# mcgillmrl/prob_mbrl

Measured on AMD Instinct MI355X. Metric: particle_rollouts_per_sec, higher is better.
Workload: dtype f32 via split fp16 (fwd, 2 pieces) / bf16 (adjoint, 2 pieces) MFMA, fp32 accumulate

## Files before the change

prob_mbrl_amd/csrc/pmbrl_reg.h:

```cpp
#pragma once
#include <cstddef>
#include <type_traits>
#include <utility>
#include "pmbrl_dev.h"
#include "pmbrl_split.h"
#include "pmbrl_reg_head.h"
#include "pmbrl_reg_mm.h"

#define PR_NTHR (PR_NW * 64)
#define PR_NT 13
#define PR_KB 7
#define PM_GLOBAL_ __attribute__((address_space(1)))
typedef float f32x2 __attribute__((ext_vector_type(2)));

#define PR_RES_FLOATS (PR_NW * PR_SLOTS * PR_KB * 2 * PR_FRAG)
#define PR_XT_FLOATS (PR_KB * 2 * PR_FRAG)
#define PR_L0P_FLOATS (PR_NT * 2 * PR_FRAG)
#define PR_L0_FLOATS (PR_NT * PR_FRAG)
#define PR_HEAD_FLOATS (PR_NW * 2 * 2 * PR_FRAG)
#define PR_NET_FLOATS (PR_RES_FLOATS + PR_XT_FLOATS + PR_L0P_FLOATS + PR_HEAD_FLOATS)
#define PR_OFF_RES 0
#define PR_OFF_XT (PR_RES_FLOATS)
#define PR_OFF_L0 (PR_RES_FLOATS + PR_XT_FLOATS)
#define PR_OFF_HEAD (PR_RES_FLOATS + PR_XT_FLOATS + PR_L0P_FLOATS)
// ... 203 lines not shown
      for (int e = 0; e < 8; ++e) {
        int ot = -1;
        if (blk == 0) ot = 4 * (e >> 2) + w;
        else if (e < 4) ot = 8 + w;
        else if (w == pr_xwave(net)) ot = PR_XT;
        const int k = ot >= 0 ? 16 * ot + 4 * g + (e & 3) : hid;
        piece[e] = p;
        if (k < hid) {
          if (dir == 0) {
            const int row = pr_head_row(net, P.D, P.U, m);
            if (row >= 0 && row < n_out) v[e] = W2[(size_t)row * hid + k];
          } else {
            const int i = 2 * (m >> 2) + ((m >> 1) & 1);
            if ((m & 1) == 0 && i < n_in) v[e] = W0[(size_t)k * n_in + i];
          }
        }
      }
    }
    unsigned short h[8];
#pragma unroll
    for (int e = 0; e < 8; ++e) {
      if (f16 && piece[e] == 0 && P.wflag && !(fabsf(v[e]) <= 65504.f)) atomicMax(P.wflag, P.gen);
      h[e] = pr_piece(v[e], piece[e], f16);
    }
    uint4 o4;
    o4.x = h[0] | ((unsigned)h[1] << 16);
    o4.y = h[2] | ((unsigned)h[3] << 16);
    o4.z = h[4] | ((unsigned)h[5] << 16);
    o4.w = h[6] | ((unsigned)h[7] << 16);
    *reinterpret_cast<uint4*>(P.out + ((size_t)dn * PR_NET_FLOATS + (size_t)fr * PR_FRAG) + lane * 4) = o4;
  }
}

__device__ __forceinline__ void pr_barrier() { asm volatile("s_waitcnt lgkmcnt(0)\n\ts_barrier" ::: "memory"); }
typedef __amdgpu_buffer_rsrc_t pr_rsrc;
__device__ __forceinline__ pr_rsrc pr_make_rsrc(void* base) {
  return __builtin_amdgcn_make_buffer_rsrc(base, 0, 0xffffffff, 0x00020000);
}
__device__ __forceinline__ int pr_uni(int v) { return __builtin_amdgcn_readfirstlane(v); }
#ifdef PR_EXP_NOSTASH
#define PR_EXP_STASH(x) ;
#else
#define PR_EXP_STASH(x) x
#endif
typedef int pr_i32x4 __attribute__((ext_vector_type(4)));
__device__ __forceinline__ pr_i32x4 pr_rsrc_words(const void* base) {
  const unsigned long long a = (unsigned long long)base;
  pr_i32x4 r;
  r[0] = __builtin_amdgcn_readfirstlane((int)(unsigned)a);
  r[1] = __builtin_amdgcn_readfirstlane((int)((unsigned)(a >> 32) & 0xffffu));
  r[2] = -1;
  r[3] = 0x00020000;
  return r;
}
__device__ __forceinline__ void pr_aload4_b8(unsigned (&d)[4], const pr_i32x4& srd, unsigned voff, int s0, int s1, int s2, int s3) {
  asm volatile("s_nop 4\n\tbuffer_load_ubyte %0, %4, %5, %6 offen\n\tbuffer_load_ubyte %1, %4, %5, %7 offen\n\t"
               "buffer_load_ubyte %2, %4, %5, %8 offen\n\tbuffer_load_ubyte %3, %4, %5, %9 offen"
               : "=&v"(d[0]), "=&v"(d[1]), "=&v"(d[2]), "=&v"(d[3])
               : "v"(voff), "s"(srd), "s"(s0), "s"(s1), "s"(s2), "s"(s3)
               : "memory");
}

#define PR_NRESF (2 * PR_SLOTS * PR_KB * 2)
#define PR_NAG 62
struct RegW {
  f32x4 a[PR_NAG];
  f32x4 v[PR_NRESF - PR_NAG];
};
__host__ __device__ constexpr int pr_widx(int net, int slot, int kb, int p) { return ((net * PR_SLOTS + slot) * PR_KB + kb) * 2 + p; }

template <int I>
__device__ __forceinline__ void pr_res_load(RegW& W, unsigned voff, const float* packed_dir, int wid) {
  typedef const PM_GLOBAL_ char* gcp;
  constexpr int net = I / (PR_SLOTS * PR_KB * 2), r = I % (PR_SLOTS * PR_KB * 2);
  gcp src = (gcp)(packed_dir + (size_t)net * PR_NET_FLOATS + PR_OFF_RES + ((size_t)wid * (PR_SLOTS * PR_KB * 2) + r) * PR_FRAG);
  if constexpr (I < PR_NAG) asm volatile("global_load_dwordx4 %0, %1, %2" : "=a"(W.a[I]) : "v"(voff), "s"(src) : "memory");
  else asm volatile("global_load_dwordx4 %0, %1, %2" : "=v"(W.v[I - PR_NAG]) : "v"(voff), "s"(src) : "memory");
}
template <int I>
__device__ __forceinline__ void pr_res_tie(RegW& W) {
  if constexpr (I < PR_NAG) asm volatile("" : "+a"(W.a[I]));
  else asm volatile("" : "+v"(W.v[I - PR_NAG]));
}
__device__ __forceinline__ void pr_load_resident(RegW& W, const float* packed_dir, int wid, int lane) {
  const unsigned voff = (unsigned)lane * 16u;
  pr_for<PR_NRESF>([&](auto ic) { pr_res_load<decltype(ic)::value>(W, voff, packed_dir, wid); });
  asm volatile("s_waitcnt vmcnt(0)" ::: "memory");
  pr_for<PR_NRESF>([&](auto ic) { pr_res_tie<decltype(ic)::value>(W); });
}

template <int NET, bool F16, bool XT>
__device__ __forceinline__ void pr_hidden_layer(const RegW& W, const float* lds, const float* xtw, int lane,
                                                f32x4 (&acc)[PR_SLOTS][2], f32x4 (&accx)[2]) {
  const float* act = lds + PR_LDS_ACT + lane * 4;
  f32x4 b[2][2];
  f32x4 xw[2][2];
  auto fetch = [&](int kb) {
    const int q = kb & 1;
    b[q][0] = *reinterpret_cast<const f32x4*>(act + (kb * 2 + 0) * PR_FRAG);
    b[q][1] = *reinterpret_cast<const f32x4*>(act + (kb * 2 + 1) * PR_FRAG);
    if constexpr (XT) {
      xw[q][0] = *reinterpret_cast<const f32x4*>(xtw + lane * 4 + (kb * 2 + 0) * PR_FRAG);
      xw[q][1] = *reinterpret_cast<const f32x4*>(xtw + lane * 4 + (kb * 2 + 1) * PR_FRAG);
    }
  };
  fetch(0);
  pr_for<PR_KB>([&](auto ic) {
    constexpr int kb = decltype(ic)::value;
    constexpr int q = kb & 1;
    if constexpr (kb + 1 < PR_KB) fetch(kb + 1);
    pr_for<PR_SLOTS>([&](auto sc) {
      constexpr int s = decltype(sc)::value;
      constexpr int I = pr_widx(NET, s, kb, 1);
      if constexpr (kb == 0) {
        if constexpr (I < PR_NAG) pr_mfma0<F16, true>(acc[s][0], W.a[I], b[q][0]);
        else pr_mfma0<F16, false>(acc[s][0], W.v[I - PR_NAG], b[q][0]);
      } else {
        if constexpr (I < PR_NAG) pr_mfma<F16, true>(acc[s][0], W.a[I], b[q][0]);
        else pr_mfma<F16, false>(acc[s][0], W.v[I - PR_NAG], b[q][0]);
      }
    });
    if constexpr (XT) {
      if constexpr (kb == 0) pr_mfma0<F16, false>(accx[0], xw[q][1], b[q][0]);
      else pr_mfma<F16, false>(accx[0], xw[q][1], b[q][0]);
    }
    pr_for<PR_SLOTS>([&](auto sc) {
      constexpr int s = decltype(sc)::value;
      constexpr int I = pr_widx(NET, s, kb, 0);
      if constexpr (kb == 0) {
        if constexpr (I < PR_NAG) pr_mfma0<F16, true>(acc[s][1], W.a[I], b[q][1]);
        else pr_mfma0<F16, false>(acc[s][1], W.v[I - PR_NAG], b[q][1]);
      } else {
        if constexpr (I < PR_NAG) pr_mfma<F16, true>(acc[s][1], W.a[I], b[q][1]);
        else pr_mfma<F16, false>(acc[s][1], W.v[I - PR_NAG], b[q][1]);
      }
    });
    if constexpr (XT) {
      if constexpr (kb == 0) pr_mfma0<F16, false>(accx[1], xw[q][0], b[q][1]);
      else pr_mfma<F16, false>(accx[1], xw[q][0], b[q][1]);
    }
    pr_for<PR_SLOTS>([&](auto sc) {
      constexpr int s = decltype(sc)::value;
      constexpr int I = pr_widx(NET, s, kb, 0);
      if constexpr (I < PR_NAG) pr_mfma<F16, true>(acc[s][1], W.a[I], b[q][0]);
      else pr_mfma<F16, false>(acc[s][1], W.v[I - PR_NAG], b[q][0]);
    });
    if constexpr (XT) pr_mfma<F16, false>(accx[1], xw[q][0], b[q][0]);
  });
  if constexpr (XT)
    asm volatile("s_nop 7\n\ts_nop 7" : "+v"(acc[0][0]), "+v"(acc[0][1]), "+v"(acc[1][0]), "+v"(acc[1][1]), "+v"(acc[2][0]),
                 "+v"(acc[2][1]), "+v"(accx[0]), "+v"(accx[1]));
  else
    asm volatile("s_nop 7\n\ts_nop 7" : "+v"(acc[0][0]), "+v"(acc[0][1]), "+v"(acc[1][0]), "+v"(acc[1][1]), "+v"(acc[2][0]),
                 "+v"(acc[2][1]));
}

template <bool F16>
__device__ __forceinline__ f32x4 pr_tile_value(const f32x4 (&c)[2]) {
  return pm_chains_sum<F16, 2>(c[0], c[1]);
}

template <bool F16>
__device__ __forceinline__ void pr_split(f32x4 h, pm_u32x2& hi, pm_u32x2& lo) {
  if constexpr (F16) {
    const unsigned ha = pm_pk_f16(h[0], h[1]), hb = pm_pk_f16(h[2], h[3]);
    float l0, l1, l2, l3;
    asm("v_fma_mix_f32 %0, %1, -1.0, %2 op_sel:[0,0,0] op_sel_hi:[1,0,0]" : "=v"(l0) : "v"(ha), "v"(h[0]));
    asm("v_fma_mix_f32 %0, %1, -1.0, %2 op_sel:[1,0,0] op_sel_hi:[1,0,0]" : "=v"(l1) : "v"(ha), "v"(h[1]));
    asm("v_fma_mix_f32 %0, %1, -1.0, %2 op_sel:[0,0,0] op_sel_hi:[1,0,0]" : "=v"(l2) : "v"(hb), "v"(h[2]));
    asm("v_fma_mix_f32 %0, %1, -1.0, %2 op_sel:[1,0,0] op_sel_hi:[1,0,0]" : "=v"(l3) : "v"(hb), "v"(h[3]));
    hi = pm_u32x2{ha, hb};
    lo = pm_u32x2{pm_pk_f16(l0, l1), pm_pk_f16(l2, l3)};
  } else {
    pm_u32x2 pc[2];
    pm_split4<2, F16>(h, pc);
    hi = pc[0];
    lo = pc[1];
  }
}

__device__ __forceinline__ float pr_rcp(float d) {
  const float r = __builtin_amdgcn_rcpf(d);
  return __builtin_fmaf(__builtin_fmaf(-d, r, 1.f), r, r);
}
__device__ __forceinline__ float pr_exp(float x) {
  const float t = x * 1.44269504f;
  const float eps = __builtin_fmaf(x, 1.92596299e-8f, __builtin_fmaf(x, 1.44269504f, -t));
  const float p = __builtin_amdgcn_exp2f(t);
  return __builtin_fmaf(p, eps * 0.693147181f, p);
}
__device__ __forceinline__ float pr_tanh(float u) {
  const float r = 1.f - 2.f * pr_rcp(1.f + pr_exp(2.f * __builtin_amdgcn_fmed3f(u, -15.f, 15.f)));
  return u != u ? u : r;
}
__device__ __forceinline__ float pr_sigmoid_neg(float y) { return pr_rcp(1.f + pr_exp(__builtin_amdgcn_fmed3f(y, -80.f, 80.f))); }

template <bool F16>
__device__ __forceinline__ void pr_tile_epilogue(f32x4 v, f32x4 mf, f32x4& h, unsigned& ab, unsigned& amax, pm_u32x2& hi,
                                                 pm_u32x2& lo) {
  const f32x4 t = v * mf;
#pragma unroll
  for (int r = 0; r < 4; ++r) h[r] = fmaxf(t[r], 0.f);
  {
    unsigned x0, x1, x2, x3;
    asm("v_min_u32 %0, 1, %1" : "=v"(x0) : "v"(__float_as_uint(h[0])));
    asm("v_min_u32 %0, 1, %1" : "=v"(x1) : "v"(__float_as_uint(h[1])));
    asm("v_min_u32 %0, 1, %1" : "=v"(x2) : "v"(__float_as_uint(h[2])));
    asm("v_min_u32 %0, 1, %1" : "=v"(x3) : "v"(__float_as_uint(h[3])));
    unsigned a01, a23;
    asm("v_lshl_or_b32 %0, %1, 1, %2" : "=v"(a01) : "v"(x1), "v"(x0));
    asm("v_lshl_or_b32 %0, %1, 1, %2" : "=v"(a23) : "v"(x3), "v"(x2));
    asm("v_lshl_or_b32 %0, %1, 2, %2" : "=v"(ab) : "v"(a23), "v"(a01));
  }
  amax = max(max(amax, max(__float_as_uint(h[0]), __float_as_uint(h[1]))), max(__float_as_uint(h[2]), __float_as_uint(h[3])));
  if constexpr (F16) {
    const unsigned ha = pm_pk_f16(h[0], h[1]), hb = pm_pk_f16(h[2], h[3]);
    float l0, l1, l2, l3;
    asm("v_fma_mix_f32 %0, %1, -1.0, %2 op_sel:[0,0,0] op_sel_hi:[1,0,0]" : "=v"(l0) : "v"(ha), "v"(h[0]));
    asm("v_fma_mix_f32 %0, %1, -1.0, %2 op_sel:[1,0,0] op_sel_hi:[1,0,0]" : "=v"(l1) : "v"(ha), "v"(h[1]));
    asm("v_fma_mix_f32 %0, %1, -1.0, %2 op_sel:[0,0,0] op_sel_hi:[1,0,0]" : "=v"(l2) : "v"(hb), "v"(h[2]));
    asm("v_fma_mix_f32 %0, %1, -1.0, %2 op_sel:[1,0,0] op_sel_hi:[1,0,0]" : "=v"(l3) : "v"(hb), "v"(h[3]));
    hi = pm_u32x2{ha, hb};
    lo = pm_u32x2{pm_pk_f16(l0, l1), pm_pk_f16(l2, l3)};
  } else {
    pm_u32x2 pc[2];
    pm_split4<2, F16>(h, pc);
    hi = pc[0];
    lo = pc[1];
  }
}

template <int L0_BLOCKS>
__device__ __forceinline__ void pr_copy_net_to_lds(float* smem, int lds_l0, int lds_xt, int lds_head, const float* src, int tid) {
  constexpr int N_L0 = PR_NT * L0_BLOCKS * PR_FRAG / 4, N_XT = PR_XT_FLOATS / 4, N_HD = PR_HEAD_FLOATS / 4;
  constexpr int I_L0 = (N_L0 + PR_NTHR - 1) / PR_NTHR, I_XT = (N_XT + PR_NTHR - 1) / PR_NTHR, I_HD = (N_HD + PR_NTHR - 1) / PR_NTHR;
  f32x4 a[I_L0], b[I_XT], c[I_HD];
#pragma unroll
  for (int k = 0; k < I_L0; ++k) {
    const int i = min(tid + k * PR_NTHR, N_L0 - 1);
    a[k] = ldg4(src + PR_OFF_L0 + (L0_BLOCKS == 1 ? (i >> 6) * (2 * PR_FRAG) + (i & 63) * 4 : i * 4));
  }
#pragma unroll
  for (int k = 0; k < I_XT; ++k) b[k] = ldg4(src + PR_OFF_XT + min(tid + k * PR_NTHR, N_XT - 1) * 4);
#pragma unroll
  for (int k = 0; k < I_HD; ++k) c[k] = ldg4(src + PR_OFF_HEAD + min(tid + k * PR_NTHR, N_HD - 1) * 4);
#pragma unroll
  for (int k = 0; k < I_L0; ++k)
    if (tid + k * PR_NTHR < N_L0) *reinterpret_cast<f32x4*>(smem + lds_l0 + (tid + k * PR_NTHR) * 4) = a[k];
#pragma unroll
  for (int k = 0; k < I_XT; ++k)
    if (tid + k * PR_NTHR < N_XT) *reinterpret_cast<f32x4*>(smem + lds_xt + (tid + k * PR_NTHR) * 4) = b[k];
#pragma unroll
  for (int k = 0; k < I_HD; ++k)
    if (tid + k * PR_NTHR < N_HD) *reinterpret_cast<f32x4*>(smem + lds_head + (tid + k * PR_NTHR) * 4) = c[k];
}

template <bool PROF, int MMD = 0, bool TREE = false>
__global__ __launch_bounds__(PR_NTHR, 1) void pm_reg_fwd_kernel(const RegArgs A) {
  extern __shared__ __attribute__((aligned(16))) float smem[];
  constexpr bool F16 = true;
  constexpr int MMDc = MMD ? MMD : 2;
  typedef PM_GLOBAL_ uint8_t gu8;
  typedef PM_GLOBAL_ float gf32;
  typedef PM_GLOBAL_ char gch;
  const int tid = threadIdx.x, lane = tid & 63;
  const int wid = __builtin_amdgcn_readfirstlane(tid >> 6);
  const int wg = pr_wg(A);
  if (wg < 0) return;
  const int row = lane & 15, g = lane >> 4;
  int row0, nvalid;
  pr_rows(A, wg, row0, nvalid);
  const bool rvalid = row < nvalid;
  const int D = A.D, U = A.U, B = A.B;
  const float* packed = A.packed;

  if (PROF && wg == 0 && tid == 0) {
    A.prof[30] = (long long)__builtin_readcyclecounter();
    A.prof[28] = (long long)__builtin_amdgcn_s_memrealtime();
  }
  float c_mx[2], c_isx[2], c_sy[2], c_my[2], c_zp[2], c_zd[2], c_psc[2], c_pbi[2];
  float x[2];
  unsigned so_x[2], so_a[2];
  bool ok_x[2], ok_a[2];
#pragma unroll
  for (int s = 0; s < 2; ++s) {
    const int i = 2 * g + s;
    const bool isd = i < D, isa = i >= D && i < D + U;
    const int ja = isa ? i - D : 0, id = isd ? i : 0;
    c_mx[s] = (isd || isa) ? A.mx[i] : 0.f;
    c_isx[s] = (isd || isa) ? A.iSx[i] : 0.f;
    c_sy[s] = isd ? A.Sy[id] : 0.f;
    c_my[s] = isd ? A.my[id] : 0.f;
    c_zp[s] = (isa && rvalid) ? A.zpol[(size_t)(row0 + row) * U + ja] : 0.f;
    c_zd[s] = (isd && rvalid) ? A.zdyn[(size_t)(row0 + row) * D + id] : 0.f;
    c_psc[s] = isa ? A.pscale[ja] : 0.f;
    c_pbi[s] = isa ? A.pbias[ja] : 0.f;
    x[s] = (isd && rvalid) ? A.x0[(size_t)(row0 + row) * D + id] : 0.f;
    ok_x[s] = isd && rvalid;
    ok_a[s] = isa && rvalid;
    so_x[s] = ((unsigned)(row0 + row) * D + id) * 4u;
    so_a[s] = ((unsigned)(row0 + row) * U + ja) * 4u;
  }
  f32x4 hbp, hbd;
#pragma unroll
  for (int r = 0; r < 4; ++r) {
    const int rp = pr_head_row(0, D, U, 4 * g + r), rd = pr_head_row(1, D, U, 4 * g + r);
    hbp[r] = rp >= 0 ? (A.pol_params + A.pol.b_off[2])[rp] : 0.f;
    hbd[r] = rd >= 0 ? (A.dyn_params + A.dyn.b_off[2])[rd] : 0.f;
  }
  unsigned mbits[2][2][PR_SLOTS + 1];
#pragma unroll
  for (int n = 0; n < 2; ++n)
#pragma unroll
    for (int l = 0; l < 2; ++l) {
      const uint16_t* mrow = (n == 0 ? A.pol : A.dyn).mask[l] + (size_t)(row0 + (rvalid ? row : 0)) * PR_NT;
#pragma unroll
      for (int q = 0; q <= PR_SLOTS; ++q) mbits[n][l][q] = (unsigned)mrow[q < PR_SLOTS ? 4 * q + wid : PR_XT];
    }
  RegW W;
  pr_load_resident(W, packed, wid, lane);
  if (PROF && wg == 0 && tid == 0) A.prof[27] = (long long)__builtin_readcyclecounter();
#pragma unroll
  for (int s = 0; s < 2; ++s)
    if (ok_x[s] && wid == 0) *(gf32*)((gch*)A.states + so_x[s]) = x[s];
  pr_copy_net_to_lds<1>(smem, PR_LDS_L0(0), PR_LDS_XT(0), PR_LDS_HEAD(0), packed, tid);
  pr_copy_net_to_lds<1>(smem, PR_LDS_L0(1), PR_LDS_XT(1), PR_LDS_HEAD(1), packed + PR_NET_FLOATS, tid);
  if (PROF && wg == 0 && tid == 0) A.prof[26] = (long long)__builtin_readcyclecounter();
  for (int i = tid; i < PR_KB * 2 * PR_FRAG; i += PR_NTHR) smem[PR_LDS_ACT + i] = 0.f;
  if (tid < 16) smem[PR_LDS_FLAG + tid] = 0.f;
#pragma unroll
  for (int n = 0; n < 2; ++n)
#pragma unroll
    for (int l = 0; l < 2; ++l) {
      const RegNet& N = n == 0 ? A.pol : A.dyn;
#pragma unroll
      for (int q = 0; q <= PR_SLOTS; ++q) {
        if (q == PR_SLOTS && wid != pr_xwave(n)) continue;
        const unsigned nib = rvalid ? ((mbits[n][l][q] >> (4 * g)) & 0xFu) : 0u;
        f32x4 mf;
#pragma unroll
        for (int r = 0; r < 4; ++r) mf[r] = ((nib >> r) & 1u) ? N.inv_keep[l] : 0.f;
        float* dst = q < PR_SLOTS ? smem + PR_LDS_MF + (size_t)(((wid * 2 + n) * 2 + l) * PR_SLOTS + q) * PR_FRAG
                                  : smem + PR_LDS_MFX + (size_t)(n * 2 + l) * PR_FRAG;
        *reinterpret_cast<f32x4*>(dst + lane * 4) = mf;
      }
    }
  __syncthreads();
  if (tid < 64) reinterpret_cast<unsigned*>(smem + PR_LDS_ACT + ((PR_KB - 1) * 2 + 0) * PR_FRAG + tid * 4)[2] = 0x3c00u;
  if (tid == 0 && A.wflag && *A.wflag == A.wgen) atomicMin(A.status, 0);
  if (PROF && wg == 0 && tid == 0) A.prof[25] = (long long)__builtin_readcyclecounter();

  bool any_a[2], any_x[2];
#pragma unroll
  for (int s = 0; s < 2; ++s) {
    any_a[s] = false;
    any_x[s] = false;
    for (int gg = 0; gg < 4; ++gg) {
      const int i = 2 * gg + s;
      any_a[s] = any_a[s] || (i >= D && i < D + U);
      any_x[s] = any_x[s] || i < D;
    }
  }
  const float max_std_pol = expf(A.mls_pol), max_std_dyn = expf(A.mls_dyn);
  const int mm_gi = MMD ? wg / A.mm.parts : 0, mm_me = MMD ? wg - mm_gi * A.mm.parts : 0, mm_g0 = mm_gi * (MMD ? A.mm.M : 0);
  double mm_ref = 0.0;
  double* const mm_zh = reinterpret_cast<double*>(smem + PR_LDS_ZH);
  double* const mm_rec = reinterpret_cast<double*>(smem + PR_LDS_REC);
  if constexpr (MMD != 0) {
    if (wid == 0) mm_ref = row < MMD ? (double)A.x0[(size_t)mm_g0 * D + row] : 0.0;
    if (wid == 1) pr_mm_fwd_prep<MMDc>(A.mm, 0, mm_gi, mm_g0, row0, nvalid, mm_me, lane, mm_zh);
  }
  unsigned amax = 0u;
  const bool xw_pol = wid == pr_xwave(0), xw_dyn = wid == pr_xwave(1);
  float* const act_w = smem + PR_LDS_ACT + lane * 4;
  const float* const mf_w = smem + PR_LDS_MF + (size_t)wid * (2 * 2 * PR_SLOTS * PR_FRAG) + lane * 4;
  const float* const mfx_w = smem + PR_LDS_MFX + lane * 4;
  const unsigned lane_st = ((4u * g) * 16u + row) * 4u;
  const pr_rsrc srd = pr_make_rsrc(A.ws);
  const unsigned vo_abp = (unsigned)lane * 4u;
  int so_abp = (wg * PR_NW + wid) * 256;
  const int abp_step = A.nwg * (PR_NW * 256);

  auto first_layer = [&](auto netc, const float (&in)[2], int so_ab, int so_st) {
    constexpr int NET = decltype(netc)::value;
    _Float16 hh[2], hl[2], hs[2];
#pragma unroll
    for (int s = 0; s < 2; ++s) {
      hh[s] = (_Float16)in[s];
      hl[s] = (_Float16)(in[s] - (float)hh[s]);
      hs[s] = hh[s] * (_Float16)PM_F16_LO_ISCALE;
      amax = max(amax, __float_as_uint(in[s]) & 0x7fffffffu);
#ifdef PR_EXP_AMAX_CODE
      if (!(fabsf(in[s]) <= 3.0e38f)) atomicMin(A.status, -((NET + 1) * 1000000 + lane * 1000 + s * 100 + wg));
#endif
    }
    const pm_f16x8 bf = {hh[0], hl[0], hs[0], hh[1], hl[1], hs[1], (_Float16)1.0f, (_Float16)PM_F16_LO_ISCALE};
    const float* l0w = smem + PR_LDS_L0(NET) + lane * 4;
    const bool xw = NET == 0 ? xw_pol : xw_dyn;
    f32x4 acc[PR_SLOTS + 1];
    const f32x4 bfv = __builtin_bit_cast(f32x4, bf);
    f32x4 wf[PR_SLOTS + 1];
    pr_for<PR_SLOTS>([&](auto qc) {
      constexpr int q = decltype(qc)::value;
      wf[q] = *reinterpret_cast<const f32x4*>(l0w + (size_t)(4 * q + wid) * PR_FRAG);
    });
    wf[PR_SLOTS] = *reinterpret_cast<const f32x4*>(l0w + (size_t)PR_XT * PR_FRAG);
    f32x4 mfv[PR_SLOTS + 1];
    pr_for<PR_SLOTS>([&](auto qc) {
      constexpr int q = decltype(qc)::value;
      mfv[q] = *reinterpret_cast<const f32x4*>(mf_w + (size_t)((NET * 2 + 0) * PR_SLOTS + q) * PR_FRAG);
    });
    mfv[PR_SLOTS] = *reinterpret_cast<const f32x4*>(mfx_w + (size_t)(NET * 2 + 0) * PR_FRAG);
    pr_mfma_open();
    pr_for<PR_SLOTS + 1>([&](auto qc) {
      constexpr int q = decltype(qc)::value;
      pr_mfma0<F16, false, true>(acc[q], wf[q], bfv);
    });
    asm volatile("s_nop 7\n\ts_nop 7" : "+v"(acc[0]), "+v"(acc[1]), "+v"(acc[2]), "+v"(acc[3]));
    unsigned abw = 0u;
    auto epi = [&](auto qc, int ot) {
      constexpr int q = decltype(qc)::value;
      f32x4 h;
      unsigned ab;
      pm_u32x2 hi, lo;
      pr_tile_epilogue<F16>(acc[q], mfv[q], h, ab, amax, hi, lo);
      float* dst = act_w + (size_t)((ot >> 1) * 2) * PR_FRAG + 2 * (ot & 1);
      *reinterpret_cast<pm_u32x2*>(dst) = hi;
      *reinterpret_cast<pm_u32x2*>(dst + PR_FRAG) = lo;
      abw |= ab << (4 * q);
      if constexpr (NET == 0) {
#pragma unroll
        for (int r = 0; r < 4; ++r)
// ... 220 lines not shown
  if (U.mm_on) {
    const int gi = wg / U.parts, me = wg - gi * U.parts;
    row0 = gi * U.M + me * U.rpw;
    nvalid = min(U.rpw, U.M - me * U.rpw);
  }
  const int rowg = row0 + (lane & 15), g = lane >> 4;
  if ((lane & 15) >= nvalid) return;
  for (int n = 0; n < 2; ++n)
    for (int l = 0; l < 2; ++l) {
      const unsigned w = U.src[n][l][((size_t)t * U.nwg + wg) * PR_NTHR + tid];
      unsigned char* d = U.dst[n][l] + ((size_t)t * U.B + rowg) * (PR_NT * 4) + g;
#pragma unroll
      for (int q = 0; q < PR_SLOTS; ++q) d[(4 * q + wid) * 4] = (unsigned char)((w >> (4 * q)) & 15u);
      if (wid == pr_xwave(n)) d[PR_XT * 4] = (unsigned char)((w >> (4 * PR_SLOTS)) & 15u);
    }
}

#define PRB_LDS_ACT 0
#define PRB_LDS_PART (PRB_LDS_ACT + PR_KB * 2 * PR_FRAG)
#define PRB_LDS_L0(net) (PRB_LDS_PART + PR_NW * PR_FRAG + (net) * (PR_L0P_FLOATS + PR_XT_FLOATS + PR_HEAD_FLOATS))
#define PRB_LDS_XT(net) (PRB_LDS_L0(net) + PR_L0P_FLOATS)
#define PRB_LDS_HEAD(net) (PRB_LDS_XT(net) + PR_XT_FLOATS)
#define PRB_LDS_LUT (PRB_LDS_L0(2))
#define PRB_IN_COLS 32
#define PRB_LDS_IN (PRB_LDS_LUT + 2 * 2 * 16 * 4)
#define PRB_LDS_XB (PRB_LDS_IN + 16 * PRB_IN_COLS)
#define PRB_LDS_MMB (PRB_LDS_XB + 128)
#define PRB_LDS_MMY (PRB_LDS_MMB + 2 * 2 * PR_MM_BOP_DOUBLES)
#define PRB_LDS_XH (PRB_LDS_MMY + 2 * 2 * PR_MM_YOP_DOUBLES(6))
#define PRB_LDS_XTAG (PRB_LDS_XH + 2 * PM_XCH_HELP_DOUBLES(2))
#define PRB_LDS_FLOATS (PRB_LDS_XTAG + 16)

template <bool PROF, int MMD = 0, bool TREE = false>
__global__ __launch_bounds__(PR_NTHR, 1) void pm_reg_bwd_kernel(const RegArgs A) {
  extern __shared__ __attribute__((aligned(16))) float smem[];
  constexpr bool F16 = false;
  constexpr int MMDc = MMD ? MMD : 2;
  typedef PM_GLOBAL_ float gf32;
  const int tid = threadIdx.x, lane = tid & 63;
  const int wid = __builtin_amdgcn_readfirstlane(tid >> 6);
  const int wg = pr_wg(A);
  if (wg < 0) return;
  const int row = lane & 15, g = lane >> 4;
  int row0, nvalid;
  pr_rows(A, wg, row0, nvalid);
  const bool rvalid = row < nvalid;
  const int D = A.D, U = A.U, B = A.B;
  const int T0 = A.t0;
  int T1 = A.t1;
  if (A.nvalid) T1 = min(T1, __builtin_amdgcn_readfirstlane(*A.nvalid));
  const float* packed = A.packed + (size_t)2 * PR_NET_FLOATS;
  if (T1 <= T0) {
    for (int i = tid; i < nvalid * D; i += PR_NTHR) {
      if (A.grad_x0 && T0 == 0) A.grad_x0[(size_t)row0 * D + i] = 0.f;
      if (A.gx_out) A.gx_out[(size_t)row0 * D + i] = A.gx_in ? A.gx_in[(size_t)row0 * D + i] : 0.f;
    }
    return;
  }

  if (PROF && wg == 0 && tid == 0) {
    A.prof[30] = (long long)__builtin_readcyclecounter();
    A.prof[28] = (long long)__builtin_amdgcn_s_memrealtime();
  }
  float c_isx[2], c_sy[2], c_psc[2], c_pbi[2];
  bool ok_x[2], ok_a[2];
  unsigned so_x[2], so_a[2];
  float gx[2] = {0.f, 0.f};
#pragma unroll
  for (int s = 0; s < 2; ++s) {
    const int i = 2 * g + s;
    const bool isd = i < D, isa = i >= D && i < D + U;
    const int ja = isa ? i - D : 0, id = isd ? i : 0;
    c_isx[s] = (isd || isa) ? A.iSx[i] : 0.f;
    c_sy[s] = isd ? A.Sy[id] : 0.f;
    c_psc[s] = isa ? A.pscale[ja] : 1.f;
    c_pbi[s] = isa ? A.pbias[ja] : 0.f;
    ok_x[s] = isd && rvalid;
    ok_a[s] = isa && rvalid;
    so_x[s] = ((unsigned)(row0 + row) * D + id) * 4u;
    so_a[s] = ((unsigned)(row0 + row) * U + ja) * 4u;
    if (A.gx_in && ok_x[s]) gx[s] = *(const gf32*)((const PM_GLOBAL_ char*)A.gx_in + so_x[s]);
  }
  RegW W;
  pr_load_resident(W, packed, wid, lane);
  pr_copy_net_to_lds<2>(smem, PRB_LDS_L0(0), PRB_LDS_XT(0), PRB_LDS_HEAD(0), packed, tid);
  pr_copy_net_to_lds<2>(smem, PRB_LDS_L0(1), PRB_LDS_XT(1), PRB_LDS_HEAD(1), packed + PR_NET_FLOATS, tid);
  for (int i = tid; i < PR_KB * 2 * PR_FRAG; i += PR_NTHR) smem[PRB_LDS_ACT + i] = 0.f;
  if (tid < 16) smem[PRB_LDS_XTAG + tid] = 0.f;
  if (tid < 64) {
    const int n = tid >> 5, l = (tid >> 4) & 1, nib = tid & 15;
    const float ik = (n == 0 ? A.pol : A.dyn).inv_keep[l];
    f32x4 m;
#pragma unroll
    for (int r = 0; r < 4; ++r) m[r] = ((nib >> r) & 1) ? ik : 0.f;
    *reinterpret_cast<f32x4*>(smem + PRB_LDS_LUT + tid * 4) = m;
  }
  __syncthreads();

  const bool xw_pol = wid == pr_xwave(0), xw_dyn = wid == pr_xwave(1);
  float* const act_w = smem + PRB_LDS_ACT + lane * 4;
  const float* const lut = smem + PRB_LDS_LUT;
  const unsigned lane_st = ((4u * g) * 16u + row) * 4u;
  const pr_rsrc srd = pr_make_rsrc(A.ws);
  const unsigned x_step = (unsigned)B * D * 4u, a_step = (unsigned)B * U * 4u;
  const int st_step = A.nwg * (PR_NT * 1024), st_step2 = A.nwg * 1024;
  int so_g0 = (int)A.gT[0] + ((T1 - 1) * A.nwg + wg) * (PR_NT * 1024);
  int so_g2 = (int)A.gT[2] + ((T1 - 1) * A.nwg + wg) * 1024;

  float* const stage = smem + PRB_LDS_IN;
  typedef const PM_GLOBAL_ char* gcp;
  gcp sp[2];
  unsigned sstep[2];
#pragma unroll
  for (int k = 0; k < 2; ++k) {
    const int e = tid + k * PR_NTHR, r = e >> 5, c = e & 31;
    const long long grow = row0 + r;
    gcp q = (gcp)A.ws;
    unsigned st = 0u;
    if (r < nvalid) {
      const int i = c >= 18 ? c - 18 : (c >= 10 ? c - 10 : c - 2);
      if (c == 0) {
        q = (gcp)A.grad_rewards + ((long long)(T1 - 1) * B + grow) * 4;
        st = (unsigned)B * 4u;
      } else if (c >= 2 && c < 26 && i < D && c < 18) {
        q = (gcp)A.ws + (c < 10 ? A.Jx : A.Td) + ((long long)(T1 - 1) * B + grow) * D * 4 + i * 4;
        st = x_step;
      } else if (c >= 2 && c < 26 && i >= D && i < D + U) {
        q = (c >= 18 ? (gcp)A.actions : (gcp)A.ws + (c < 10 ? A.Ja : A.Tp)) + ((long long)(T1 - 1) * B + grow) * U * 4 + (i - D) * 4;
        st = a_step;
      }
    }
    sp[k] = q;
    sstep[k] = st;
  }
  float sv[2];
  auto stage_load = [&]() {
    asm volatile("global_load_dword %0, %2, off\n\tglobal_load_dword %1, %3, off" : "=&v"(sv[0]), "=&v"(sv[1]) : "v"(sp[0]), "v"(sp[1]) : "memory");
  };
  auto stage_landed = [&](auto nc, float (&v)[2]) {
    constexpr int N = decltype(nc)::value;
    asm volatile("s_waitcnt vmcnt(%2)" : "+v"(v[0]), "+v"(v[1]) : "n"(N) : "memory");
  };
  auto stage_park = [&]() {
    stage[tid] = sv[0];
    stage[tid + PR_NTHR] = sv[1];
  };
  const pr_i32x4 wsrd = pr_rsrc_words(A.ws);
  const unsigned vo_abp = (unsigned)lane * 4u;
  const int abp_step = A.nwg * (PR_NW * 256);
  int so_abp = ((T1 - 1) * A.nwg + wg) * (PR_NW * 256) + wid * 256;
  auto ab_load = [&](unsigned (&w)[4]) {
    asm volatile("s_nop 4\n\tbuffer_load_dword %0, %4, %5, %6 offen\n\tbuffer_load_dword %1, %4, %5, %7 offen\n\t"
                 "buffer_load_dword %2, %4, %5, %8 offen\n\tbuffer_load_dword %3, %4, %5, %9 offen"
                 : "=&v"(w[0]), "=&v"(w[1]), "=&v"(w[2]), "=&v"(w[3])
                 : "v"(vo_abp), "s"(wsrd), "s"(pr_uni((int)A.dyn.abits[1] + so_abp)), "s"(pr_uni((int)A.dyn.abits[0] + so_abp)),
                   "s"(pr_uni((int)A.pol.abits[1] + so_abp)), "s"(pr_uni((int)A.pol.abits[0] + so_abp))
                 : "memory");
  };
  auto ab_landed = [&](auto nc, unsigned (&w)[4]) {
    constexpr int N = decltype(nc)::value;
    asm volatile("s_waitcnt vmcnt(%4)" : "+v"(w[0]), "+v"(w[1]), "+v"(w[2]), "+v"(w[3]) : "n"(N) : "memory");
  };
  const float* const st_row = stage + row * PRB_IN_COLS;
  struct StepIn {
    float gr, jx[2], td[2];
  };
  auto read_in = [&](StepIn& I) {
    const f32x2 a = *reinterpret_cast<const f32x2*>(st_row + 2 + 2 * g), b = *reinterpret_cast<const f32x2*>(st_row + 10 + 2 * g);
    I.gr = rvalid ? st_row[0] : 0.f;
#pragma unroll
    for (int s = 0; s < 2; ++s) {
      I.jx[s] = ok_x[s] ? a[s] : 0.f;
      I.td[s] = ok_x[s] ? b[s] : 0.f;
    }
  };

  auto head_adjoint = [&](auto netc, const float (&gm)[2], const float (&gl)[2], const unsigned abw) {
    constexpr int NET = decltype(netc)::value;
    f32x4 bf[2];
    PR_HEAD_BFRAGS(gm, gl, bf)
// ... 17 lines not shown
      pr_mfma<F16, false, true>(acc[q], wf[q][1], bf[1]);
    });
    asm volatile("s_nop 7\n\ts_nop 7" : "+v"(acc[0]), "+v"(acc[1]), "+v"(acc[2]), "+v"(acc[3]));
    auto epi = [&](auto qc, int ot) {
      constexpr int q = decltype(qc)::value;
      const f32x4 gq = acc[q] * mfv[q];
      pm_u32x2 pc[2];
      pm_split4<2, false>(gq, pc);
      float* dst = act_w + (size_t)((ot >> 1) * 2) * PR_FRAG + 2 * (ot & 1);
      *reinterpret_cast<pm_u32x2*>(dst) = pc[0];
      *reinterpret_cast<pm_u32x2*>(dst + PR_FRAG) = pc[1];
    };
    pr_for<PR_SLOTS>([&](auto qc) {
      constexpr int q = decltype(qc)::value;
      epi(qc, 4 * q + wid);
    });
    if (xw) epi(std::integral_constant<int, PR_SLOTS>{}, PR_XT);
  };

  auto hidden_adjoint_and_tail = [&](auto netc, const unsigned abw, int so_st, f32x4& o, auto arrived) {
    constexpr int NET = decltype(netc)::value;
    const bool xw = NET == 0 ? xw_pol : xw_dyn;
    f32x4 acc[PR_SLOTS][2], accx[2];
    f32x4 mfv[PR_SLOTS + 1], hwv[2][2];
    if (xw) pr_hidden_layer<NET, F16, true>(W, smem, smem + PRB_LDS_XT(NET), lane, acc, accx);
    else pr_hidden_layer<NET, F16, false>(W, smem, nullptr, lane, acc, accx);
    arrived();
    pr_for<PR_SLOTS + 1>([&](auto qc) {
      constexpr int q = decltype(qc)::value;
      mfv[q] = *reinterpret_cast<const f32x4*>(lut + ((NET * 2 + 0) * 16 + ((abw >> (4 * q)) & 15u)) * 4);
    });
    const float* hw = smem + PRB_LDS_HEAD(NET) + (size_t)wid * (4 * PR_FRAG) + lane * 4;
#pragma unroll
    for (int blkk = 0; blkk < 2; ++blkk) {
      hwv[blkk][0] = *reinterpret_cast<const f32x4*>(hw + (blkk * 2 + 0) * PR_FRAG);
      hwv[blkk][1] = *reinterpret_cast<const f32x4*>(hw + (blkk * 2 + 1) * PR_FRAG);
    }
    pm_u32x2 hi[PR_SLOTS + 1], lo[PR_SLOTS + 1];
    hi[PR_SLOTS] = lo[PR_SLOTS] = pm_u32x2{0u, 0u};
    auto epi = [&](auto qc, f32x4 v, int ot) {
      constexpr int q = decltype(qc)::value;
      const f32x4 gq = v * mfv[q];
      pm_u32x2 pc[2];
      pm_split4<2, false>(gq, pc);
      hi[q] = pc[0];
      lo[q] = pc[1];
      if constexpr (NET == 0) {
#pragma unroll
        for (int r = 0; r < 4; ++r)
          PR_EXP_STASH(__builtin_amdgcn_raw_buffer_store_b32(__float_as_uint(gq[r]), srd, lane_st + r * 64, pr_uni(so_st + ot * 1024), 0);)
      }
    };
    pr_for<PR_SLOTS>([&](auto qc) {
      constexpr int q = decltype(qc)::value;
      epi(qc, pr_tile_value<F16>(acc[q]), 4 * q + wid);
    });
    if (xw) epi(std::integral_constant<int, PR_SLOTS>{}, pr_tile_value<F16>(accx), PR_XT);
    f32x4 c0, c1, bh[2], bl[2];
#pragma unroll
    for (int blkk = 0; blkk < 2; ++blkk) {
      const pm_u32x2 ha = hi[2 * blkk], hb = hi[2 * blkk + 1], la = lo[2 * blkk], lb = lo[2 * blkk + 1];
      bh[blkk] = __builtin_bit_cast(f32x4, (pr_u32x4){ha[0], ha[1], hb[0], hb[1]});
      bl[blkk] = __builtin_bit_cast(f32x4, (pr_u32x4){la[0], la[1], lb[0], lb[1]});
    }
    pr_mfma_open();
    pr_mfma0<F16, false, true>(c0, hwv[0][1], bh[0]);
    pr_mfma0<F16, false, true>(c1, hwv[0][0], bl[0]);
    pr_mfma<F16, false, true>(c0, hwv[1][1], bh[1]);
    pr_mfma<F16, false, true>(c1, hwv[0][0], bh[0]);
    pr_mfma<F16, false, true>(c1, hwv[1][0], bl[1]);
    pr_mfma<F16, false, true>(c1, hwv[1][0], bh[1]);
    asm volatile("s_nop 7\n\ts_nop 7" : "+v"(c0), "+v"(c1));
    float* part = smem + PRB_LDS_PART + lane * 4;
    *reinterpret_cast<f32x4*>(part + wid * PR_FRAG) = c0 + c1;
    pr_barrier();
    o = *reinterpret_cast<const f32x4*>(part);
#pragma unroll
    for (int w = 1; w < PR_NW; ++w) o += *reinterpret_cast<const f32x4*>(part + w * PR_FRAG);
  };

  const int mm_gi = MMD ? wg / A.mm.parts : 0, mm_me = MMD ? wg - mm_gi * A.mm.parts : 0, mm_g0 = mm_gi * (MMD ? A.mm.M : 0);
  double* const mm_bop = reinterpret_cast<double*>(smem + PRB_LDS_MMB);
  double* const mm_yop = reinterpret_cast<double*>(smem + PRB_LDS_MMY);
  if constexpr (MMD != 0) {
    if (wid == 1) pr_mm_bwd_prep_noise<MMDc>(A.mm, T1 - 1, mm_gi, mm_g0, row0, nvalid, lane, mm_bop + ((T1 - 1) & 1) * PR_MM_BOP_DOUBLES);
    if (wid == 2) pr_mm_bwd_prep_factor<MMDc>(A.mm, B, T1 - 1, mm_gi, row0, nvalid, lane, mm_yop + ((T1 - 1) & 1) * PR_MM_YOP_DOUBLES(MMDc));
  }
  unsigned abc[4], abn[4];
  stage_load();
  ab_load(abc);
  stage_landed(std::integral_constant<int, 0>{}, sv);
  ab_landed(std::integral_constant<int, 0>{}, abc);
  stage_park();
  __syncthreads();
  for (int t = T1 - 1; t >= T0; --t) {
    if (PROF && wg == 0 && tid == 0) A.prof[(size_t)t * 32 + 0] = (long long)__builtin_readcyclecounter();
    StepIn In;
    read_in(In);
    if constexpr (MMD != 0) {
      const bool do_chain = t < T1 - 1 || A.gx_in;
      int ln = lane;
      asm volatile("" : "+v"(ln));
      pr_mm_kptr Qp = pr_mm_args();
      asm volatile("" : "+s"(Qp));
      const RegMM Q = pr_mm_load(Qp);
      if (PROF && wg == 0 && tid == 0) A.prof[(size_t)t * 32 + 6] = (long long)__builtin_readcyclecounter();
      if (wid == 1 && t > T0) {
        pr_mm_bwd_prep_noise<MMDc>(Q, t - 1, mm_gi, mm_g0, row0, nvalid, ln, mm_bop + ((t - 1) & 1) * PR_MM_BOP_DOUBLES);
        if (PROF && wg == 0 && lane == 0) A.prof[(size_t)t * 32 + 13] = (long long)__builtin_readcyclecounter();
      } else if (wid == 2 && t > T0) {
        pr_mm_bwd_prep_factor<MMDc>(Q, B, t - 1, mm_gi, row0, nvalid, ln, mm_yop + ((t - 1) & 1) * PR_MM_YOP_DOUBLES(MMDc));
        if (PROF && wg == 0 && lane == 0) A.prof[(size_t)t * 32 + 14] = (long long)__builtin_readcyclecounter();
      }
      if (do_chain) {
        double* const xh = reinterpret_cast<double*>(smem + PRB_LDS_XH);
        volatile unsigned* const xtag = reinterpret_cast<volatile unsigned*>(smem + PRB_LDS_XTAG);
        if constexpr (TREE) {
          if (wid != 0) {
            const bool okh = pm_xch_tree_help<PR_MM_NVX(MMDc), 4>(Q.xch, Q.nwg, mm_gi * Q.parts, Q.parts, Q.fan, mm_me, Q.tag0 + (unsigned)(T1 - t), wid, xh,
                                                    xtag, ln);
            if (!okh && lane == 0 && A.status) atomicMax(A.status, 1);
          }
        }
        if (wid == 0) {
          float go[(MMDc + 3) / 4];
          const bool ok = pr_mm_bwd_chain<MMDc, TREE>(Q, Q.tag0 + (unsigned)(T1 - t), mm_me, mm_gi * Q.parts, nvalid, ln, gx,
                                                 mm_bop + (t & 1) * PR_MM_BOP_DOUBLES, mm_yop + (t & 1) * PR_MM_YOP_DOUBLES(MMDc), go,
                                                 xh, xtag, (PROF && wg <= 1) ? A.prof + (size_t)t * 32 + 8 * wg : nullptr);
          if (!ok && lane == 0 && A.status) atomicMax(A.status, 1);
#pragma unroll
          for (int rr = 0; rr < (MMDc + 3) / 4; ++rr) smem[PRB_LDS_XB + row * 8 + g + 4 * rr] = go[rr];
        }
        pr_barrier();
        const f32x2 gm = *reinterpret_cast<const f32x2*>(smem + PRB_LDS_XB + row * 8 + 2 * g);
#pragma unroll
        for (int s = 0; s < 2; ++s) gx[s] = ok_x[s] ? gm[s] : 0.f;
        if (PROF && wg == 0 && tid == 0) A.prof[(size_t)t * 32 + 7] = (long long)__builtin_readcyclecounter();
      }
    }
    if (t > T0) {
#pragma unroll
      for (int k = 0; k < 2; ++k) sp[k] -= sstep[k];
      so_abp -= abp_step;
    }
    stage_load();
    ab_load(abn);
    float gxn[2], gm[2], gl[2];
#pragma unroll
    for (int s = 0; s < 2; ++s) {
      const float gg = gx[s] + In.gr * In.jx[s];
      gxn[s] = gg;
      gm[s] = gg * c_sy[s];
      gl[s] = gg * In.td[s];
    }
    head_adjoint(std::integral_constant<int, 1>{}, gm, gl, abc[0]);
    pr_barrier();
    if (PROF && wg == 0 && tid == 0) A.prof[(size_t)t * 32 + 1] = (long long)__builtin_readcyclecounter();
    f32x4 o;
    hidden_adjoint_and_tail(std::integral_constant<int, 1>{}, abc[1], 0, o, []() {});
    if (PROF && wg == 0 && tid == 0) A.prof[(size_t)t * 32 + 2] = (long long)__builtin_readcyclecounter();
    float pm_[2], pl_[2];
    {
      const f32x2 ja = *reinterpret_cast<const f32x2*>(st_row + 2 + 2 * g), tp = *reinterpret_cast<const f32x2*>(st_row + 10 + 2 * g),
                  ac = *reinterpret_cast<const f32x2*>(st_row + 18 + 2 * g);
#pragma unroll
      for (int s = 0; s < 2; ++s) {
        const float tail = o[2 * s] * c_isx[s];
        gxn[s] += ok_x[s] ? tail : 0.f;
        const float ga = In.gr * (ok_a[s] ? ja[s] : 0.f) + tail;
        const float th = ((ok_a[s] ? ac[s] : c_pbi[s]) - c_pbi[s]) * pr_rcp(c_psc[s]);
        const float gu = ok_a[s] ? ga * c_psc[s] * (1.f - th * th) : 0.f;
        pm_[s] = gu;
        pl_[s] = ok_a[s] ? gu * tp[s] : 0.f;
      }
    }
    if (wid == 2) {
#pragma unroll
// ... 58 lines not shown
```

Before: 6.415 million.

## Overlap kernel prologue weight loads with LDS staging via split vmcnt waits

The prologue of the forward and adjoint kernels is restructured so that all global loads are issued up front. These cover the LDS-bound net sections, the resident AGPR and VGPR weight fragments, the x0, wflag and mask words, and the backward stage and ab inputs. Waits use partial vmcnt counts so the LDS sections can be parked while the VGPR weights are still in flight. The goal is to cut serialized prologue latency before the time loop. The cost is more hand-managed inline asm and vmcnt bookkeeping, which is fragile if load counts change.

```diff
diff --git a/prob_mbrl_amd/csrc/pmbrl_reg.h b/prob_mbrl_amd/csrc/pmbrl_reg.h
--- a/prob_mbrl_amd/csrc/pmbrl_reg.h
+++ b/prob_mbrl_amd/csrc/pmbrl_reg.h
@@ -309,9 +309,19 @@
   if constexpr (I < PR_NAG) asm volatile("" : "+a"(W.a[I]));
   else asm volatile("" : "+v"(W.v[I - PR_NAG]));
 }
-__device__ __forceinline__ void pr_load_resident(RegW& W, const float* packed_dir, int wid, int lane) {
+__device__ __forceinline__ void pr_request_agprs(RegW& W, const float* packed_dir, int wid, int lane) {
   const unsigned voff = (unsigned)lane * 16u;
-  pr_for<PR_NRESF>([&](auto ic) { pr_res_load<decltype(ic)::value>(W, voff, packed_dir, wid); });
+  pr_for<PR_NAG>([&](auto ic) { pr_res_load<decltype(ic)::value>(W, voff, packed_dir, wid); });
+}
+__device__ __forceinline__ void pr_landed_but_agprs() {
+  static_assert(PR_NAG <= 63, "the vm counter's field");
+  asm volatile("s_waitcnt vmcnt(%0)" ::"n"(PR_NAG) : "memory");
+}
+__device__ __forceinline__ void pr_request_vgprs(RegW& W, const float* packed_dir, int wid, int lane) {
+  const unsigned voff = (unsigned)lane * 16u;
+  pr_for<PR_NRESF - PR_NAG>([&](auto ic) { pr_res_load<PR_NAG + decltype(ic)::value>(W, voff, packed_dir, wid); });
+}
+__device__ __forceinline__ void pr_landed_all(RegW& W) {
   asm volatile("s_waitcnt vmcnt(0)" ::: "memory");
   pr_for<PR_NRESF>([&](auto ic) { pr_res_tie<decltype(ic)::value>(W); });
 }
@@ -458,28 +468,56 @@
 }
 
 template <int L0_BLOCKS>
-__device__ __forceinline__ void pr_copy_net_to_lds(float* smem, int lds_l0, int lds_xt, int lds_head, const float* src, int tid) {
-  constexpr int N_L0 = PR_NT * L0_BLOCKS * PR_FRAG / 4, N_XT = PR_XT_FLOATS / 4, N_HD = PR_HEAD_FLOATS / 4;
-  constexpr int I_L0 = (N_L0 + PR_NTHR - 1) / PR_NTHR, I_XT = (N_XT + PR_NTHR - 1) / PR_NTHR, I_HD = (N_HD + PR_NTHR - 1) / PR_NTHR;
+struct PrSect {
+  static constexpr int N_L0 = PR_NT * L0_BLOCKS * PR_FRAG / 4, N_XT = PR_XT_FLOATS / 4, N_HD = PR_HEAD_FLOATS / 4;
+  static constexpr int I_L0 = (N_L0 + PR_NTHR - 1) / PR_NTHR, I_XT = (N_XT + PR_NTHR - 1) / PR_NTHR, I_HD = (N_HD + PR_NTHR - 1) / PR_NTHR;
   f32x4 a[I_L0], b[I_XT], c[I_HD];
-#pragma unroll
-  for (int k = 0; k < I_L0; ++k) {
-    const int i = min(tid + k * PR_NTHR, N_L0 - 1);
-    a[k] = ldg4(src + PR_OFF_L0 + (L0_BLOCKS == 1 ? (i >> 6) * (2 * PR_FRAG) + (i & 63) * 4 : i * 4));
-  }
-#pragma unroll
-  for (int k = 0; k < I_XT; ++k) b[k] = ldg4(src + PR_OFF_XT + min(tid + k * PR_NTHR, N_XT - 1) * 4);
-#pragma unroll
-  for (int k = 0; k < I_HD; ++k) c[k] = ldg4(src + PR_OFF_HEAD + min(tid + k * PR_NTHR, N_HD - 1) * 4);
-#pragma unroll
-  for (int k = 0; k < I_L0; ++k)
-    if (tid + k * PR_NTHR < N_L0) *reinterpret_cast<f32x4*>(smem + lds_l0 + (tid + k * PR_NTHR) * 4) = a[k];
-#pragma unroll
-  for (int k = 0; k < I_XT; ++k)
-    if (tid + k * PR_NTHR < N_XT) *reinterpret_cast<f32x4*>(smem + lds_xt + (tid + k * PR_NTHR) * 4) = b[k];
-#pragma unroll
-  for (int k = 0; k < I_HD; ++k)
-    if (tid + k * PR_NTHR < N_HD) *reinterpret_cast<f32x4*>(smem + lds_head + (tid + k * PR_NTHR) * 4) = c[k];
+};
+__device__ __forceinline__ void pr_sect_load(f32x4& d, const float* src, int float_off) {
+  typedef const PM_GLOBAL_ char* gcp;
+  asm volatile("global_load_dwordx4 %0, %1, %2" : "=v"(d) : "v"((unsigned)float_off * 4u), "s"((gcp)src) : "memory");
+}
+__device__ __forceinline__ void pr_sect_tie(f32x4& d) { asm volatile("" : "+v"(d)); }
+template <int L0_BLOCKS>
+__device__ __forceinline__ void pr_sect_request(PrSect<L0_BLOCKS>& S, const float* src, int tid) {
+  typedef PrSect<L0_BLOCKS> P;
+  pr_for<P::I_L0>([&](auto kc) {
+    constexpr int k = decltype(kc)::value;
+    const int i = min(tid + k * PR_NTHR, P::N_L0 - 1);
+    pr_sect_load(S.a[k], src, PR_OFF_L0 + (L0_BLOCKS == 1 ? (i >> 6) * (2 * PR_FRAG) + (i & 63) * 4 : i * 4));
+  });
+  pr_for<P::I_XT>([&](auto kc) {
+    constexpr int k = decltype(kc)::value;
+    pr_sect_load(S.b[k], src, PR_OFF_XT + min(tid + k * PR_NTHR, P::N_XT - 1) * 4);
+  });
+  pr_for<P::I_HD>([&](auto kc) {
+    constexpr int k = decltype(kc)::value;
+    pr_sect_load(S.c[k], src, PR_OFF_HEAD + min(tid + k * PR_NTHR, P::N_HD - 1) * 4);
+  });
+}
+template <int L0_BLOCKS>
+__device__ __forceinline__ void pr_sect_park(PrSect<L0_BLOCKS>& S, float* smem, int lds_l0, int lds_xt, int lds_head, int tid) {
+  typedef PrSect<L0_BLOCKS> P;
+#pragma unroll
+  for (int k = 0; k < P::I_L0; ++k) pr_sect_tie(S.a[k]);
+#pragma unroll
+  for (int k = 0; k < P::I_XT; ++k) pr_sect_tie(S.b[k]);
+#pragma unroll
+  for (int k = 0; k < P::I_HD; ++k) pr_sect_tie(S.c[k]);
+#pragma unroll
+  for (int k = 0; k < P::I_L0; ++k)
+    if (tid + k * PR_NTHR < P::N_L0) *reinterpret_cast<f32x4*>(smem + lds_l0 + (tid + k * PR_NTHR) * 4) = S.a[k];
+#pragma unroll
+  for (int k = 0; k < P::I_XT; ++k)
+    if (tid + k * PR_NTHR < P::N_XT) *reinterpret_cast<f32x4*>(smem + lds_xt + (tid + k * PR_NTHR) * 4) = S.b[k];
+#pragma unroll
+  for (int k = 0; k < P::I_HD; ++k)
+    if (tid + k * PR_NTHR < P::N_HD) *reinterpret_cast<f32x4*>(smem + lds_head + (tid + k * PR_NTHR) * 4) = S.c[k];
+}
+
+template <int BYTES>
+__device__ __forceinline__ void pr_mask_load(unsigned& d, unsigned voff, const PM_GLOBAL_ char* base) {
+  asm volatile("global_load_ushort %0, %1, %2 offset:%3" : "=v"(d) : "v"(voff), "s"(base), "n"(BYTES) : "memory");
 }
 
 template <bool PROF, int MMD = 0, bool TREE = false>
@@ -506,7 +544,6 @@
     A.prof[28] = (long long)__builtin_amdgcn_s_memrealtime();
   }
   float c_mx[2], c_isx[2], c_sy[2], c_my[2], c_zp[2], c_zd[2], c_psc[2], c_pbi[2];
-  float x[2];
   unsigned so_x[2], so_a[2];
   bool ok_x[2], ok_a[2];
 #pragma unroll
@@ -522,7 +559,6 @@
     c_zd[s] = (isd && rvalid) ? A.zdyn[(size_t)(row0 + row) * D + id] : 0.f;
     c_psc[s] = isa ? A.pscale[ja] : 0.f;
     c_pbi[s] = isa ? A.pbias[ja] : 0.f;
-    x[s] = (isd && rvalid) ? A.x0[(size_t)(row0 + row) * D + id] : 0.f;
     ok_x[s] = isd && rvalid;
     ok_a[s] = isa && rvalid;
     so_x[s] = ((unsigned)(row0 + row) * D + id) * 4u;
@@ -535,25 +571,52 @@
     hbp[r] = rp >= 0 ? (A.pol_params + A.pol.b_off[2])[rp] : 0.f;
     hbd[r] = rd >= 0 ? (A.dyn_params + A.dyn.b_off[2])[rd] : 0.f;
   }
+  typedef const PM_GLOBAL_ char* gcc;
+  float xl[2];
+#pragma unroll
+  for (int s = 0; s < 2; ++s)
+    asm volatile("global_load_dword %0, %1, %2" : "=v"(xl[s]) : "v"(ok_x[s] ? so_x[s] : (unsigned)row0 * D * 4u), "s"((gcc)A.x0) : "memory");
+  unsigned wfl;
+  asm volatile("global_load_dword %0, %1, %2" : "=v"(wfl) : "v"(0u), "s"(A.wflag ? (gcc)A.wflag : (gcc)A.x0) : "memory");
   unsigned mbits[2][2][PR_SLOTS + 1];
-#pragma unroll
-  for (int n = 0; n < 2; ++n)
-#pragma unroll
-    for (int l = 0; l < 2; ++l) {
-      const uint16_t* mrow = (n == 0 ? A.pol : A.dyn).mask[l] + (size_t)(row0 + (rvalid ? row : 0)) * PR_NT;
-#pragma unroll
-      for (int q = 0; q <= PR_SLOTS; ++q) mbits[n][l][q] = (unsigned)mrow[q < PR_SLOTS ? 4 * q + wid : PR_XT];
-    }
+  {
+    const unsigned mo_row = (unsigned)(row0 + (rvalid ? row : 0)) * (PR_NT * 2u);
+    const unsigned mo_w = mo_row + (unsigned)wid * 2u, mo_x = mo_row + PR_XT * 2u;
+#pragma unroll
+    for (int n = 0; n < 2; ++n)
+#pragma unroll
+      for (int l = 0; l < 2; ++l) {
+        gcc mbase = (gcc)(n == 0 ? A.pol : A.dyn).mask[l];
+        static_assert(PR_SLOTS == 3, "mask words of the resident tiles 4 q + wid");
+        pr_mask_load<0>(mbits[n][l][0], mo_w, mbase);
+        pr_mask_load<8>(mbits[n][l][1], mo_w, mbase);
+        pr_mask_load<16>(mbits[n][l][2], mo_w, mbase);
+        pr_mask_load<0>(mbits[n][l][PR_SLOTS], mo_x, mbase);
+      }
+  }
   RegW W;
-  pr_load_resident(W, packed, wid, lane);
-  if (PROF && wg == 0 && tid == 0) A.prof[27] = (long long)__builtin_readcyclecounter();
-#pragma unroll
-  for (int s = 0; s < 2; ++s)
+  {
+    PrSect<1> sp_, sd_;
+    pr_sect_request(sp_, packed, tid);
+    pr_sect_request(sd_, packed + PR_NET_FLOATS, tid);
+    pr_request_agprs(W, packed, wid, lane);
+    pr_landed_but_agprs();
+    if (PROF && wg == 0 && tid == 0) A.prof[27] = (long long)__builtin_readcyclecounter();
+    pr_sect_park(sp_, smem, PR_LDS_L0(0), PR_LDS_XT(0), PR_LDS_HEAD(0), tid);
+    pr_sect_park(sd_, smem, PR_LDS_L0(1), PR_LDS_XT(1), PR_LDS_HEAD(1), tid);
+  }
+  pr_request_vgprs(W, packed, wid, lane);
+  asm volatile("" : "+v"(xl[0]), "+v"(xl[1]), "+v"(wfl));
+  float x[2];
+#pragma unroll
+  for (int s = 0; s < 2; ++s) {
+    x[s] = ok_x[s] ? xl[s] : 0.f;
     if (ok_x[s] && wid == 0) *(gf32*)((gch*)A.states + so_x[s]) = x[s];
-  pr_copy_net_to_lds<1>(smem, PR_LDS_L0(0), PR_LDS_XT(0), PR_LDS_HEAD(0), packed, tid);
-  pr_copy_net_to_lds<1>(smem, PR_LDS_L0(1), PR_LDS_XT(1), PR_LDS_HEAD(1), packed + PR_NET_FLOATS, tid);
-  if (PROF && wg == 0 && tid == 0) A.prof[26] = (long long)__builtin_readcyclecounter();
-  for (int i = tid; i < PR_KB * 2 * PR_FRAG; i += PR_NTHR) smem[PR_LDS_ACT + i] = 0.f;
+  }
+  for (int i = tid; i < PR_KB * 2 * PR_FRAG; i += PR_NTHR) {
+    const int j = i - ((PR_KB - 1) * 2 + 0) * PR_FRAG;
+    reinterpret_cast<unsigned*>(smem + PR_LDS_ACT)[i] = (j >= 0 && j < PR_FRAG && (j & 3) == 2) ? 0x3c00u : 0u;
+  }
   if (tid < 16) smem[PR_LDS_FLAG + tid] = 0.f;
 #pragma unroll
   for (int n = 0; n < 2; ++n)
@@ -562,6 +625,7 @@
       const RegNet& N = n == 0 ? A.pol : A.dyn;
 #pragma unroll
       for (int q = 0; q <= PR_SLOTS; ++q) {
+        asm volatile("" : "+v"(mbits[n][l][q]));
         if (q == PR_SLOTS && wid != pr_xwave(n)) continue;
         const unsigned nib = rvalid ? ((mbits[n][l][q] >> (4 * g)) & 0xFu) : 0u;
         f32x4 mf;
@@ -572,9 +636,10 @@
         *reinterpret_cast<f32x4*>(dst + lane * 4) = mf;
       }
     }
+  pr_landed_all(W);
+  if (PROF && wg == 0 && tid == 0) A.prof[26] = (long long)__builtin_readcyclecounter();
   __syncthreads();
-  if (tid < 64) reinterpret_cast<unsigned*>(smem + PR_LDS_ACT + ((PR_KB - 1) * 2 + 0) * PR_FRAG + tid * 4)[2] = 0x3c00u;
-  if (tid == 0 && A.wflag && *A.wflag == A.wgen) atomicMin(A.status, 0);
+  if (tid == 0 && A.wflag && (int)wfl == A.wgen) atomicMin(A.status, 0);
   if (PROF && wg == 0 && tid == 0) A.prof[25] = (long long)__builtin_readcyclecounter();
 
   bool any_a[2], any_x[2];
@@ -961,20 +1026,6 @@
     if (A.gx_in && ok_x[s]) gx[s] = *(const gf32*)((const PM_GLOBAL_ char*)A.gx_in + so_x[s]);
   }
   RegW W;
-  pr_load_resident(W, packed, wid, lane);
-  pr_copy_net_to_lds<2>(smem, PRB_LDS_L0(0), PRB_LDS_XT(0), PRB_LDS_HEAD(0), packed, tid);
-  pr_copy_net_to_lds<2>(smem, PRB_LDS_L0(1), PRB_LDS_XT(1), PRB_LDS_HEAD(1), packed + PR_NET_FLOATS, tid);
-  for (int i = tid; i < PR_KB * 2 * PR_FRAG; i += PR_NTHR) smem[PRB_LDS_ACT + i] = 0.f;
-  if (tid < 16) smem[PRB_LDS_XTAG + tid] = 0.f;
-  if (tid < 64) {
-    const int n = tid >> 5, l = (tid >> 4) & 1, nib = tid & 15;
-    const float ik = (n == 0 ? A.pol : A.dyn).inv_keep[l];
-    f32x4 m;
-#pragma unroll
-    for (int r = 0; r < 4; ++r) m[r] = ((nib >> r) & 1) ? ik : 0.f;
-    *reinterpret_cast<f32x4*>(smem + PRB_LDS_LUT + tid * 4) = m;
-  }
-  __syncthreads();
 
   const bool xw_pol = wid == pr_xwave(0), xw_dyn = wid == pr_xwave(1);
   float* const act_w = smem + PRB_LDS_ACT + lane * 4;
@@ -1158,17 +1209,41 @@
   const int mm_gi = MMD ? wg / A.mm.parts : 0, mm_me = MMD ? wg - mm_gi * A.mm.parts : 0, mm_g0 = mm_gi * (MMD ? A.mm.M : 0);
   double* const mm_bop = reinterpret_cast<double*>(smem + PRB_LDS_MMB);
   double* const mm_yop = reinterpret_cast<double*>(smem + PRB_LDS_MMY);
+  unsigned abc[4], abn[4];
+  stage_load();
+  ab_load(abc);
+  {
+    PrSect<2> sp_, sd_;
+    pr_sect_request(sp_, packed, tid);
+    pr_sect_request(sd_, packed + PR_NET_FLOATS, tid);
+    pr_request_agprs(W, packed, wid, lane);
+    pr_landed_but_agprs();
+    if (PROF && wg == 0 && tid == 0) A.prof[27] = (long long)__builtin_readcyclecounter();
+    pr_sect_park(sp_, smem, PRB_LDS_L0(0), PRB_LDS_XT(0), PRB_LDS_HEAD(0), tid);
+    pr_sect_park(sd_, smem, PRB_LDS_L0(1), PRB_LDS_XT(1), PRB_LDS_HEAD(1), tid);
+  }
+  pr_request_vgprs(W, packed, wid, lane);
+  stage_landed(std::integral_constant<int, PR_NAG>{}, sv);
+  ab_landed(std::integral_constant<int, PR_NAG>{}, abc);
+  stage_park();
+  for (int i = tid; i < PR_KB * 2 * PR_FRAG; i += PR_NTHR) smem[PRB_LDS_ACT + i] = 0.f;
+  if (tid < 16) smem[PRB_LDS_XTAG + tid] = 0.f;
+  if (tid < 64) {
+    const int n = tid >> 5, l = (tid >> 4) & 1, nib = tid & 15;
+    const float ik = n == 0 ? (l == 0 ? A.pol.inv_keep[0] : A.pol.inv_keep[1]) : (l == 0 ? A.dyn.inv_keep[0] : A.dyn.inv_keep[1]);
+    f32x4 m;
+#pragma unroll
+    for (int r = 0; r < 4; ++r) m[r] = ((nib >> r) & 1) ? ik : 0.f;
+    *reinterpret_cast<f32x4*>(smem + PRB_LDS_LUT + tid * 4) = m;
+  }
+  pr_landed_all(W);
+  if (PROF && wg == 0 && tid == 0) A.prof[26] = (long long)__builtin_readcyclecounter();
   if constexpr (MMD != 0) {
     if (wid == 1) pr_mm_bwd_prep_noise<MMDc>(A.mm, T1 - 1, mm_gi, mm_g0, row0, nvalid, lane, mm_bop + ((T1 - 1) & 1) * PR_MM_BOP_DOUBLES);
     if (wid == 2) pr_mm_bwd_prep_factor<MMDc>(A.mm, B, T1 - 1, mm_gi, row0, nvalid, lane, mm_yop + ((T1 - 1) & 1) * PR_MM_YOP_DOUBLES(MMDc));
   }
-  unsigned abc[4], abn[4];
-  stage_load();
-  ab_load(abc);
-  stage_landed(std::integral_constant<int, 0>{}, sv);
-  ab_landed(std::integral_constant<int, 0>{}, abc);
-  stage_park();
   __syncthreads();
+  if (PROF && wg == 0 && tid == 0) A.prof[25] = (long long)__builtin_readcyclecounter();
   for (int t = T1 - 1; t >= T0; --t) {
     if (PROF && wg == 0 && tid == 0) A.prof[(size_t)t * 32 + 0] = (long long)__builtin_readcyclecounter();
     StepIn In;
```

Result: no change. 6.456 million (median of 6 runs) (+0.6%).
